# chrg127/stereomatching

Hardware: AMD Instinct MI355X
Metric: Mpixel-disparities/s (higher is better)
Workload: dtype u32 bit-packed edges, i32 counts

## Files before the change

stereomatching_amd/csrc/sm_match_bs_kernel.h:

```cpp

#pragma once
#include "sm_internal.h"

#ifndef SM_BS_TU
#error "define SM_BS_TU (a token naming the translation unit) before including this header"
#endif
#define SM_BS_CAT2(a, b) a##b
#define SM_BS_CAT(a, b) SM_BS_CAT2(a, b)

#define SM_BS_WAVES 2

#ifdef SM_STAMPS
static __device__ unsigned long long *g_sm_stamps;
int SM_BS_CAT(sm_bs_set_stamps_, SM_BS_TU)(void *buf)
{
    return hipMemcpyToSymbol(HIP_SYMBOL(g_sm_stamps), &buf, sizeof buf) == hipSuccess ? 0 : SM_ERR_HIP;
}
#define SM_STAMP(slot)                                                                          \
    do {                                                                                        \
        if ((threadIdx.x & 63) == 0 && g_sm_stamps) {                   \
            const size_t wg_ = (((size_t)blockIdx.z * gridDim.y + blockIdx.y) * gridDim.x + blockIdx.x) \
                               * (blockDim.x >> 6) + (threadIdx.x >> 6);                        \
            g_sm_stamps[wg_ * 10 + 2 * (slot)] = __builtin_amdgcn_s_memrealtime();              \
            g_sm_stamps[wg_ * 10 + 2 * (slot) + 1] = __builtin_amdgcn_s_memtime();              \
            if ((slot) == 0)                                                                    \
                g_sm_stamps[wg_ * 10 + 8] = ((unsigned long long)__builtin_amdgcn_s_getreg(63508) << 32) | \
                                            (unsigned)__builtin_amdgcn_s_getreg(63492);         \
        }                                                                                       \
    } while (0)
#else
#define SM_STAMP(slot) do { } while (0)
#endif

template <int IMM>
__device__ __forceinline__ u32 bop(u32 a, u32 b, u32 c)
{
    return __builtin_amdgcn_bitop3_b32(a, b, c, IMM);
}
#define BOP_XOR3 0x96
#define BOP_MAJ 0xE8
#define BOP_BORROW 0x8E
#define BOP_SEL 0xCA
#define BOP_XOR_AND 0x28
#define BOP_UPD 0x41

__device__ __forceinline__ u32 alignbit(u32 hi, u32 lo, u32 sh)
{
    return __builtin_amdgcn_alignbit(hi, lo, sh);
}

typedef unsigned long long u64;
struct RawRow { u64 l01; u32 l2; u64 r01, r23; };
struct RawCentre { u32 l; u64 r01; u32 r2; };
typedef __attribute__((address_space(3))) const volatile u32 lds_vu32;
typedef u64 __attribute__((aligned(4))) u64a4;
typedef __attribute__((address_space(3))) const volatile u64a4 lds_vu64;
__device__ __forceinline__ void lds_issue(RawRow &o, u32 aL, u32 aR)
{
    o.l01 = *(lds_vu64 *)(uintptr_t)aL;
    o.l2 = *(lds_vu32 *)(uintptr_t)(aL + 8);
    o.r01 = *(lds_vu64 *)(uintptr_t)aR;
    o.r23 = *(lds_vu64 *)(uintptr_t)(aR + 8);
}
__device__ __forceinline__ void lds_issue(RawCentre &o, u32 aL, u32 aR)
{
    o.l = *(lds_vu32 *)(uintptr_t)aL;
    o.r01 = *(lds_vu64 *)(uintptr_t)aR;
    o.r2 = *(lds_vu32 *)(uintptr_t)(aR + 8);
}

typedef int v4i __attribute__((ext_vector_type(4)));
__device__ __forceinline__ void store_map4(i32 *p, v4i v)
{
    asm volatile("global_store_dwordx4 %0, %1, off sc1\n\ts_nop 1" : : "v"(p), "v"(v) : "memory");
}

constexpr int bits_for(int v) { int b = 0; while ((1 << b) <= v) b++; return b; }

template <int SB, int HB>
__device__ __forceinline__ void add_planes(u32 (&s)[SB], const u32 (&h)[HB])
{
    u32 c = s[0] & h[0];
    s[0] ^= h[0];
#pragma unroll
    for (int k = 1; k < SB; k++) {
        if (k < HB) {
            const u32 cn = bop<BOP_MAJ>(s[k], h[k], c);
            s[k] = bop<BOP_XOR3>(s[k], h[k], c);
            c = cn;
        } else {
            const u32 cn = k + 1 < SB ? s[k] & c : 0u;
            s[k] ^= c;
            c = cn;
        }
    }
}

#define SM_PIN() __builtin_amdgcn_sched_barrier(0)
#define SM_SYNC() do { asm volatile("s_nop 0"); SM_PIN(); } while (0)
#define BOP_ANDN 0x0C
#define BOP_ORN 0xCF
#define BOP_XNOR 0xC3

template <int N, int HB, int IT, typename XF>
__device__ __forceinline__ void count_lockstep(XF xin, u32 (&h)[IT][HB])
{
    u32 q[IT][2 * N + 2];
    int head = 0, tail = N;
#pragma unroll
    for (int w = 0; w < HB; w++) {
        u32 nx[IT][N + 1];
        int nn = 0;
#pragma unroll
        for (int adder = 0; adder < N; adder++) {
            if (tail - head >= 3) {
                u32 a[IT], b[IT], c[IT];
#pragma unroll
                for (int it = 0; it < IT; it++) {
                    const bool in0 = w == 0 && head < N, in1 = w == 0 && head + 1 < N, in2 = w == 0 && head + 2 < N;
                    a[it] = in0 ? xin(it, in0 ? head : 0) : q[it][head];
                    b[it] = in1 ? xin(it, in1 ? head + 1 : 0) : q[it][head + 1];
                    c[it] = in2 ? xin(it, in2 ? head + 2 : 0) : q[it][head + 2];
                }
#pragma unroll
                for (int it = 0; it < IT; it++) { q[it][tail] = bop<BOP_XOR3>(a[it], b[it], c[it]); SM_PIN(); }
#pragma unroll
                for (int it = 0; it < IT; it++) { nx[it][nn] = bop<BOP_MAJ>(a[it], b[it], c[it]); SM_PIN(); }
                SM_SYNC();
                head += 3; tail++; nn++;
            }
        }
        if (tail - head == 2) {
            u32 a[IT], b[IT];
#pragma unroll
            for (int it = 0; it < IT; it++) {
                const bool in0 = w == 0 && head < N, in1 = w == 0 && head + 1 < N;
                a[it] = in0 ? xin(it, in0 ? head : 0) : q[it][head];
                b[it] = in1 ? xin(it, in1 ? head + 1 : 0) : q[it][head + 1];
            }
#pragma unroll
            for (int it = 0; it < IT; it++) { q[it][tail] = a[it] ^ b[it]; SM_PIN(); }
#pragma unroll
            for (int it = 0; it < IT; it++) { nx[it][nn] = a[it] & b[it]; SM_PIN(); }
            head += 2; tail++; nn++;
        }
#pragma unroll
        for (int it = 0; it < IT; it++) {
            const bool in0 = w == 0 && head < N;
            h[it][w] = tail - head == 1 ? (in0 ? xin(it, in0 ? head : 0) : q[it][head]) : 0u;
        }
        head = 0; tail = 0;
#pragma unroll
        for (int i = 0; i < N + 1; i++)
            if (i < nn) {
#pragma unroll
                for (int it = 0; it < IT; it++) q[it][tail] = nx[it][i];
                tail++;
            }
    }
}

template <int SB, int HB, int GS, int DS>
__device__ __forceinline__ void add_lockstep(u32 (&S)[DS][SB], int dd0, const u32 (&h)[GS][HB])
{
    u32 c[GS];
#pragma unroll
    for (int g = 0; g < GS; g++) { c[g] = S[dd0 + g][0] & h[g][0]; SM_PIN(); }
#pragma unroll
    for (int g = 0; g < GS; g++) { S[dd0 + g][0] ^= h[g][0]; SM_PIN(); }
#pragma unroll
    for (int k = 1; k < SB; k++) {
        u32 cn[GS];
#pragma unroll
        for (int g = 0; g < GS; g++) {
            if (k + 1 < SB) { cn[g] = k < HB ? bop<BOP_MAJ>(S[dd0 + g][k], h[g][k], c[g]) : (S[dd0 + g][k] & c[g]); SM_PIN(); }
            else cn[g] = 0;
        }
#pragma unroll
        for (int g = 0; g < GS; g++) {
            if (k < HB) S[dd0 + g][k] = bop<BOP_XOR3>(S[dd0 + g][k], h[g][k], c[g]);
            else S[dd0 + g][k] ^= c[g];
            SM_PIN();
        }
#pragma unroll
        for (int g = 0; g < GS; g++) c[g] = cn[g];
        SM_SYNC();
    }
}

template <int SB, int HB, int GS, int DS>
__device__ __forceinline__ void addsub_lockstep(u32 (&S)[DS][SB], int dd0, const u32 (&hn)[GS][HB],
                                                const u32 (&ho)[GS][HB])
{
    u32 dl[GS][HB], b[GS];
#pragma unroll
    for (int g = 0; g < GS; g++) { b[g] = bop<BOP_ANDN>(hn[g][0], ho[g][0], 0u); SM_PIN(); }
#pragma unroll
    for (int g = 0; g < GS; g++) { dl[g][0] = hn[g][0] ^ ho[g][0]; SM_PIN(); }
#pragma unroll
    for (int k = 1; k < HB; k++) {
#pragma unroll
        for (int g = 0; g < GS; g++) { dl[g][k] = bop<BOP_XOR3>(hn[g][k], ho[g][k], b[g]); SM_PIN(); }
#pragma unroll
        for (int g = 0; g < GS; g++) { b[g] = bop<BOP_BORROW>(hn[g][k], ho[g][k], b[g]); SM_PIN(); }
        SM_SYNC();
    }
    u32 c[GS];
#pragma unroll
    for (int g = 0; g < GS; g++) { c[g] = S[dd0 + g][0] & dl[g][0]; SM_PIN(); }
#pragma unroll
    for (int g = 0; g < GS; g++) { S[dd0 + g][0] ^= dl[g][0]; SM_PIN(); }
#pragma unroll
    for (int k = 1; k < SB; k++) {
        u32 cn[GS];
#pragma unroll
        for (int g = 0; g < GS; g++) {
            const u32 a = k < HB ? dl[g][k] : b[g];
            if (k + 1 < SB) { cn[g] = bop<BOP_MAJ>(S[dd0 + g][k], a, c[g]); SM_PIN(); } else cn[g] = 0;
        }
#pragma unroll
        for (int g = 0; g < GS; g++) {
            const u32 a = k < HB ? dl[g][k] : b[g];
            S[dd0 + g][k] = bop<BOP_XOR3>(S[dd0 + g][k], a, c[g]); SM_PIN();
        }
#pragma unroll
        for (int g = 0; g < GS; g++) c[g] = cn[g];
        SM_SYNC();
    }
}

template <int V> struct IntTag { static constexpr int value = V; };

template <int CTRL>
__device__ __forceinline__ u32 dpp(u32 v)
{
    return (u32)__builtin_amdgcn_update_dpp(0, (int)v, CTRL, 0xf, 0xf, true);
}

template <int K>
__device__ __forceinline__ u32 from_partner(u32 v)
{
    if (K == 0) return dpp<0xB1>(v);
    if (K == 1) return dpp<0x4E>(v);
    if (K == 2) return dpp<0x141>(v);
    if (K == 3) return dpp<0x140>(v);
    return (u32)__shfl_xor((int)v, 1 << K);
}


template <int N, int DS, bool FULLD, bool GHOST, bool CAP2 = false, bool DUO = false>
__global__ __launch_bounds__(DUO ? 128 : 64, SM_BS_WAVES) void k_match_bs(const u32 *__restrict__ ext,
                                                 i32 *__restrict__ web, i32 *__restrict__ best,
                                                 const MatchGeom g)
{
    constexpr int HALF = N / 2;
    constexpr int HB = bits_for(N);
    constexpr int SB = bits_for(N * N);
    constexpr int AB = DS == 16 ? 4 : DS == 8 ? 3 : 2;
    constexpr int ABMAX = AB + 6;
    static_assert(SB <= 16, "window counts are moved through two byte lanes");
    static_assert((1 << SB) - 1 > N * N, "the all-ones marker must not be a real count");
    static_assert(N + DS - 1 + 31 < 96, "right window must fit three words");

    extern __shared__ __attribute__((aligned(16))) u32 lds[];
    if (CAP2) asm volatile("" ::: "v175");
    if (web == nullptr) return;
    const int tid = DUO ? (int)(threadIdx.x & 63u) : (int)threadIdx.x;
    const int wv = DUO ? __builtin_amdgcn_readfirstlane((int)(threadIdx.x >> 6)) : 0;
    const int pair = blockIdx.z;
    SM_STAMP(0);
    const unsigned slot_parity = __builtin_amdgcn_s_getreg(63492) & 1;
    unsigned long long clk = __builtin_amdgcn_s_memtime();
    constexpr unsigned PATTERN = DS == 16 ? 0xF0F0F0F0u : 0xAAAAAAAAu;
    const unsigned long long clk0 = clk;
#define SM_SLICE_PRIO()                                                               \
    do {                                                                              \
        const unsigned unit_ = (unsigned)((clk - clk0) >> 14) & 31u;                  \
        if (((PATTERN >> unit_) ^ slot_parity) & 1) __builtin_amdgcn_s_setprio(3);    \
        else __builtin_amdgcn_s_setprio(0);                                           \
    } while (0)
#define SM_SLICE_READ() do { clk = __builtin_amdgcn_s_memtime(); } while (0)
    int tile_x, tile_y;
    sm_xcd_tile(g.tiles_x, g.tiles_y, tile_x, tile_y);
    const int tx0 = tile_x * g.tw;
    const int ty0 = tile_y * (DUO ? 2 * g.tile_h : g.tile_h);
    const int plw = g.plw, prw = g.prw, nsr = g.nsr;
    const u32 *extL = ext + (size_t)pair * 2 * g.ext_image_words;
    const u32 *extR = extL + g.ext_image_words;
    u32 *pL = lds;
    u32 *pR = pL + nsr * plw;

    {
        const int wx0 = tx0 >> 5;
        const int per_row = plw + prw;
        for (int it = threadIdx.x; it < nsr * per_row; it += DUO ? 128 : 64) {
            const int row = it / per_row, k = it - row * per_row;
            const bool is_r = k >= plw;
            const int kk = is_r ? k - plw : k;
            const u32 v = (is_r ? extR : extL)[(size_t)(ty0 + row) * g.ext_words + wx0 + kk];
            if (is_r) pR[row * prw + kk] = v; else pL[row * plw + kk] = v;
        }
    }
    __syncthreads();
    SM_STAMP(1);

    const int s = tid & (g.nl - 1);
    const int wi = tid >> g.log2nl;
    const int d0 = s * DS;
    const int x0 = tx0 + 32 * wi;
    const int bL = SM_PADT + 32 * wi - HALF, bR = bL + d0;
    const int wL = bL >> 5, shL = bL & 31, wR = bR >> 5, shR = bR & 31;
    const int bRc = SM_PADT + 32 * wi + d0;
    const int wRc = bRc >> 5, shRc = bRc & 31;
    const int wLc = 1 + wi;

    u32 cvv[N];
    if (GHOST) {
        const int lo = min(64, max(0, HALF - x0)), hi = min(64, max(0, g.w + HALF - x0));
        const unsigned long long below_hi = hi >= 64 ? ~0ull : (1ull << hi) - 1ull;
        const unsigned long long below_lo = lo >= 64 ? ~0ull : (1ull << lo) - 1ull;
        const unsigned long long cm = hi > lo ? below_hi & ~below_lo : 0ull;
        const u32 c0 = (u32)cm, c1 = (u32)(cm >> 32);
#pragma unroll
        for (int i = 0; i < N; i++) cvv[i] = i ? alignbit(c1, c0, i) : c0;
    }
    u32 dvalid = (1u << DS) - 1u;
    if (!FULLD) {
        const int dlim = g.D - d0;
        dvalid = dlim >= DS ? (1u << DS) - 1u : (dlim <= 0 ? 0u : ((1u << dlim) - 1u));
    }

    u32 S[DS][SB];
#pragma unroll
    for (int dd = 0; dd < DS; dd++)
#pragma unroll
        for (int k = 0; k < SB; k++) S[dd][k] = 0;

    struct RowViews { u32 lv[N]; u32 rw[3]; };
    auto load_views = [&](int srow, RowViews &v) {
        const u32 *rl = pL + srow * plw + wL;
        const u32 *rr = pR + srow * prw + wR;
        const u32 l0 = alignbit(rl[1], rl[0], shL), l1 = alignbit(rl[2], rl[1], shL);
#pragma unroll
        for (int k = 0; k < 3; k++) v.rw[k] = alignbit(rr[k + 1], rr[k], shR);
#pragma unroll
        for (int i = 0; i < N; i++) v.lv[i] = i ? alignbit(l1, l0, i) : l0;
    };
    auto views_of = [&](const RawRow &q, RowViews &v) {
        const u32 a0 = (u32)q.l01, a1 = (u32)(q.l01 >> 32), a2 = q.l2;
        const u32 r0 = (u32)q.r01, r1 = (u32)(q.r01 >> 32), r2 = (u32)q.r23, r3 = (u32)(q.r23 >> 32);
        const u32 l0 = alignbit(a1, a0, shL), l1 = alignbit(a2, a1, shL);
        v.rw[0] = alignbit(r1, r0, shR); v.rw[1] = alignbit(r2, r1, shR); v.rw[2] = alignbit(r3, r2, shR);
#pragma unroll
        for (int i = 0; i < N; i++) v.lv[i] = i ? alignbit(l1, l0, i) : l0;
    };
    auto rview = [&](const RowViews &v, int j) -> u32 {
        return (j & 31) ? alignbit(v.rw[(j >> 5) + 1], v.rw[j >> 5], j & 31) : v.rw[j >> 5];
    };

    constexpr int GW = DS >= 4 ? 4 : DS;
    constexpr int GS = 2;
    static_assert(DS % GW == 0 && DS % GS == 0, "shift groups");
    auto slide_in = [&](int srow) {
        RowViews v;
        load_views(srow, v);
        u32 rv[N + GW - 1];
#pragma unroll
        for (int m = 0; m < N - 1; m++) rv[m + GW] = rview(v, m);
#pragma unroll
        for (int dd0 = 0; dd0 < DS; dd0 += GW) {
#pragma unroll
            for (int m = 0; m < N - 1; m++) rv[m] = rv[m + GW];
#pragma unroll
            for (int m = 0; m < GW; m++) { rv[N - 1 + m] = rview(v, dd0 + N - 1 + m); SM_PIN(); }
            SM_SYNC();
            u32 h[GW][HB];
            count_lockstep<N, HB, GW>([&](int it, int i) -> u32 {
                const u32 x = GHOST ? bop<BOP_XOR_AND>(v.lv[i], rv[it + i], cvv[i]) : (v.lv[i] ^ rv[it + i]);
                SM_PIN();
                return x;
            }, h);
            add_lockstep<SB, HB, GW, DS>(S, dd0, h);
        }
    };
    auto slide_views = [&](const RowViews &vn, const RowViews &vo) {
        u32 rn[N + GS - 1], ro[N + GS - 1];
#pragma unroll
        for (int m = 0; m < N - 1; m++) { rn[m + GS] = rview(vn, m); ro[m + GS] = rview(vo, m); }
#pragma unroll
        for (int dd0 = 0; dd0 < DS; dd0 += GS) {
#pragma unroll
            for (int m = 0; m < N - 1; m++) { rn[m] = rn[m + GS]; ro[m] = ro[m + GS]; }
#pragma unroll
            for (int m = 0; m < GS; m++) {
                rn[N - 1 + m] = rview(vn, dd0 + N - 1 + m); SM_PIN();
                ro[N - 1 + m] = rview(vo, dd0 + N - 1 + m); SM_PIN();
            }
            SM_SYNC();
            u32 h[2 * GS][HB];
            count_lockstep<N, HB, 2 * GS>([&](int it, int i) -> u32 {
                const u32 l = (it & 1) ? vo.lv[i] : vn.lv[i];
                const u32 r = (it & 1) ? ro[(it >> 1) + i] : rn[(it >> 1) + i];
                const u32 x = GHOST ? bop<BOP_XOR_AND>(l, r, cvv[i]) : (l ^ r);
                SM_PIN();
                return x;
            }, h);
            u32 hn[GS][HB], ho[GS][HB];
#pragma unroll
            for (int gq = 0; gq < GS; gq++)
#pragma unroll
                for (int k = 0; k < HB; k++) { hn[gq][k] = h[2 * gq][k]; ho[gq][k] = h[2 * gq + 1][k]; }
            addsub_lockstep<SB, HB, GS, DS>(S, dd0, hn, ho);
            SM_SYNC();
        }
    };

    const int mid = DUO ? min(ty0 + g.tile_h, g.h) : 0;
    const int sgn = DUO ? (wv ? 1 : -1) : 1;
    const int y0 = DUO ? (wv ? mid : mid - 1) : ty0;
    const int c0 = DUO ? y0 - ty0 + HALF : HALF;
    const int rows_out = DUO ? (wv ? min(ty0 + 2 * g.tile_h, g.h) - mid : mid - ty0)
                             : min(g.tile_h, g.h - ty0);

    SM_SLICE_PRIO();
    if (DUO) {
#pragma unroll 1
        for (int e = 0; e <= HALF; e++) {
        if (e == HALF) {
        constexpr int DH = DS / 2, XP = DH * SB / 2;
        static_assert(DS % 2 == 0 && (DH * SB) % 2 == 0, "exchange halves");
        typedef u32 v2u __attribute__((ext_vector_type(2)));
        v2u *xq = reinterpret_cast<v2u *>(lds + g.xm_off - XP * 128) + tid;
        auto exchange = [&](auto own_tag) {
            constexpr int OWN = decltype(own_tag)::value, OTH = 1 - OWN;
            v2u *slot_own = xq + OWN * XP * 64, *slot_oth = xq + OTH * XP * 64;
#pragma unroll
            for (int j = 0; j < XP; j++) {
                const int p = 2 * j, q = 2 * j + 1;
                const v2u v = {S[OTH * DH + p / SB][p % SB], S[OTH * DH + q / SB][q % SB]};
                slot_oth[j * 64] = v;
            }
            __syncthreads();
#pragma unroll
            for (int dd = 0; dd < DH; dd += 2) {
                u32 o[2][SB];
#pragma unroll
                for (int j = 0; j < SB; j++) {
                    const int p = 2 * j, q = 2 * j + 1;
                    const v2u v = slot_own[(dd * SB / 2 + j) * 64];
                    o[p / SB][p % SB] = v.x;
                    o[q / SB][q % SB] = v.y;
                }
                add_planes<SB, SB>(S[OWN * DH + dd], o[0]);
                add_planes<SB, SB>(S[OWN * DH + dd + 1], o[1]);
#pragma unroll
                for (int j = 0; j < SB; j++) {
                    const int p = 2 * j, q = 2 * j + 1;
                    const v2u v = {S[OWN * DH + dd + p / SB][p % SB], S[OWN * DH + dd + q / SB][q % SB]};
                    slot_own[(dd * SB / 2 + j) * 64] = v;
                }
            }
            __syncthreads();
#pragma unroll
            for (int j = 0; j < XP; j++) {
                const int p = 2 * j, q = 2 * j + 1;
                const v2u v = slot_oth[j * 64];
                S[OTH * DH + p / SB][p % SB] = v.x;
                S[OTH * DH + q / SB][q % SB] = v.y;
            }
        };
        if (wv) exchange(IntTag<1>{}); else exchange(IntTag<0>{});
        }
        slide_in(c0 + sgn * e);
        }
        if (rows_out <= 0) return;
    } else {
#pragma unroll 1
        for (int e = 0; e < N; e++) slide_in(e);
    }
    SM_SLICE_READ();
    SM_STAMP(2);

    u32 *xm_base = lds + g.xm_off - ((DUO && wv) ? g.xm_words : 0);
    u32 *xm_wbase = xm_base + (s & 3) * ((SB + AB + 3) / 4) * 256;
    const u32 xm_wunit = (u32)(wi * (g.nl >> 2) + (s >> 2) + 2 * (s & 3));
    const u32 ldsL = (u32)(uintptr_t)pL, ldsR = (u32)(uintptr_t)pR;
    const u32 sL = (u32)(sgn * 4 * plw), sR = (u32)(sgn * 4 * prw);
    u32 aNewL = ldsL + 4u * wL + sL * (HALF + 1) + 4u * plw * c0, aNewR = ldsR + 4u * wR + sR * (HALF + 1) + 4u * prw * c0;
    u32 aCenL = ldsL + 4u * wLc + 4u * plw * c0, aCenR = ldsR + 4u * wRc + 4u * prw * c0;
    RawRow qn, qo;
    RawCentre qc;
    lds_issue(qc, aCenL, aCenR);
    if (!DUO || rows_out > 1) {
        lds_issue(qn, aNewL, aNewR);
        lds_issue(qo, aNewL - sL * N, aNewR - sR * N);
    }
#pragma unroll 1
    for (int t = 0;;) {
        SM_SLICE_PRIO();
        const int y = y0 + sgn * t;
        const u32 lc = qc.l;
        const u32 c0_ = (u32)qc.r01, c1_ = (u32)(qc.r01 >> 32), c2_ = qc.r2;
        const u32 rc0 = alignbit(c1_, c0_, shRc), rc1 = alignbit(c2_, c1_, shRc);

        u32 B[SB], arg[ABMAX];
#pragma unroll
        for (int k = 0; k < ABMAX; k++) arg[k] = 0;
        {
            constexpr int Q = 4, QS = DS / Q;
            constexpr int AQ = AB - 2;
            u32 Bq[Q][SB], aq[Q][AQ > 0 ? AQ : 1];
#pragma unroll
            for (int i = 0; i < QS; i++) {
                u32 upd[Q];
                u32 rcd[Q];
#pragma unroll
                for (int qd = 0; qd < Q; qd++) {
                    const int dd = qd * QS + i;
                    rcd[qd] = dd ? alignbit(rc1, rc0, dd) : rc0; SM_PIN();
                }
                SM_SYNC();
                if (i == 0) {
#pragma unroll
                    for (int qd = 0; qd < Q; qd++) {
                        upd[qd] = bop<BOP_XNOR>(lc, rcd[qd], 0u); SM_PIN();
                        if (!FULLD) { upd[qd] &= (u32)__builtin_amdgcn_sbfe((int)dvalid, qd * QS + i, 1); SM_PIN(); }
                    }
#pragma unroll
                    for (int k = 0; k < SB; k++)
#pragma unroll
                        for (int qd = 0; qd < Q; qd++) { Bq[qd][k] = bop<BOP_ORN>(upd[qd], S[qd * QS + i][k], 0u); SM_PIN(); }
#pragma unroll
                    for (int a = 0; a < AQ; a++)
#pragma unroll
                        for (int qd = 0; qd < Q; qd++) aq[qd][a] = 0;
                } else {
                    u32 bw[Q];
#pragma unroll
                    for (int k = 0; k < SB; k++)
#pragma unroll
                        for (int qd = 0; qd < Q; qd++) {
                            bw[qd] = bop<BOP_BORROW>(Bq[qd][k], S[qd * QS + i][k], k ? bw[qd] : 0u); SM_PIN();
                            if (qd == Q - 1 && (k & 1)) SM_SYNC();
                        }
#pragma unroll
                    for (int qd = 0; qd < Q; qd++) {
                        upd[qd] = bop<BOP_UPD>(lc, rcd[qd], bw[qd]); SM_PIN();
                        if (!FULLD) { upd[qd] &= (u32)__builtin_amdgcn_sbfe((int)dvalid, qd * QS + i, 1); SM_PIN(); }
                    }
#pragma unroll
                    for (int k = 0; k < SB; k++)
#pragma unroll
                        for (int qd = 0; qd < Q; qd++) {
                            Bq[qd][k] = bop<BOP_SEL>(upd[qd], S[qd * QS + i][k], Bq[qd][k]); SM_PIN();
                            if (qd == Q - 1 && (k & 1)) SM_SYNC();
                        }
#pragma unroll
                    for (int a = 0; a < AQ; a++)
#pragma unroll
                        for (int qd = 0; qd < Q; qd++) {
                            if ((i >> a) & 1) aq[qd][a] |= upd[qd]; else aq[qd][a] = bop<BOP_ANDN>(upd[qd], aq[qd][a], 0u);
                            SM_PIN();
                        }
                }
            }
            u32 bwm[2] = {0, 0};
#pragma unroll
            for (int k = 0; k < SB; k++)
#pragma unroll
                for (int m = 0; m < 2; m++) {
                    bwm[m] = bop<BOP_BORROW>(Bq[2 * m][k], Bq[2 * m + 1][k], k ? bwm[m] : 0u); SM_PIN();
                }
            u32 Bh[2][SB], ah[2][AQ + 1];
            u32 bwf = 0;
#pragma unroll
            for (int k = 0; k < SB; k++) {
#pragma unroll
                for (int m = 0; m < 2; m++) { Bh[m][k] = bop<BOP_SEL>(bwm[m], Bq[2 * m][k], Bq[2 * m + 1][k]); SM_PIN(); }
                if (k < AQ) {
#pragma unroll
                    for (int m = 0; m < 2; m++) { ah[m][k] = bop<BOP_SEL>(bwm[m], aq[2 * m][k], aq[2 * m + 1][k]); SM_PIN(); }
                }
                if (k > 0) { bwf = bop<BOP_BORROW>(Bh[0][k - 1], Bh[1][k - 1], k > 1 ? bwf : 0u); SM_PIN(); }
            }
#pragma unroll
            for (int k = SB; k < AQ; k++)
#pragma unroll
                for (int m = 0; m < 2; m++) { ah[m][k] = bop<BOP_SEL>(bwm[m], aq[2 * m][k], aq[2 * m + 1][k]); SM_PIN(); }
            ah[0][AQ] = ~bwm[0]; SM_PIN();
            ah[1][AQ] = ~bwm[1]; SM_PIN();
            bwf = bop<BOP_BORROW>(Bh[0][SB - 1], Bh[1][SB - 1], SB > 1 ? bwf : 0u); SM_PIN();
#pragma unroll
            for (int k = 0; k < SB; k++) { B[k] = bop<BOP_SEL>(bwf, Bh[0][k], Bh[1][k]); SM_PIN(); }
#pragma unroll
            for (int k = 0; k <= AQ; k++) { arg[k] = bop<BOP_SEL>(bwf, ah[0][k], ah[1][k]); SM_PIN(); }
            arg[AQ + 1] = ~bwf; SM_PIN();
        }

        auto emit_pixels = [&](u32 (&B)[SB], u32 (&arg)[ABMAX], int xw, int yy, int pfirst, int per, int pstep) {
            const int cw = per < 4 ? per : 4;
            const u32 cmask = (1u << cw) - 1u;
            u32 allone = B[0];
#pragma unroll
            for (int k = 1; k < SB; k++) allone &= B[k];
            u32 dm1 = (u32)(g.D - 1);
            asm volatile("" : "+s"(dm1));
#pragma unroll
            for (int k = 0; k < ABMAX; k++) {
                if (k >= AB && k >= AB + g.log2nl) continue;
                arg[k] = bop<BOP_SEL>(allone, (u32)-(i32)((dm1 >> k) & 1u), arg[k]);
            }
            for (int c = 0, p0 = pfirst; c < per; c += 4, p0 += pstep) {
                u32 bb = 0, bhi = 0, alo = 0, ahi = 0;
                if (best) {
#pragma unroll
                    for (int k = 0; k < SB; k++) {
                        const u32 sp = __umul24((B[k] >> p0) & cmask, 0x204081u) & 0x01010101u;
                        if (k < 8) bb += sp << k; else bhi += sp << (k - 8);
                    }
                }
#pragma unroll
                for (int k = 0; k < ABMAX; k++) {
                    if (k >= AB && k >= AB + g.log2nl) continue;
                    const u32 sp = __umul24((arg[k] >> p0) & cmask, 0x204081u) & 0x01010101u;
                    if (k < 8) alo += sp << k; else ahi += sp << (k - 8);
                }
                const u32 none = __umul24((allone >> p0) & cmask, 0x204081u) & 0x01010101u;
                i32 wv[4], bv[4];
#pragma unroll
                for (int q = 0; q < 4; q++) {
                    const bool no = (none >> (8 * q)) & 1u;
                    int taps = N * N;
                    if (GHOST) {
                        const int x = xw + p0 + q;
                        const int cols = min(g.w - 1, x + HALF) - max(0, x - HALF) + 1;
                        const int rws = min(g.h - 1, yy + HALF) - max(0, yy - HALF) + 1;
                        taps = cols * rws;
                    }
                    const i32 a = (i32)(((alo >> (8 * q)) & 255u) | (((ahi >> (8 * q)) & 255u) << 8));
                    wv[q] = a + 1;
                    bv[q] = no ? 0 : taps - (i32)(((bb >> (8 * q)) & 255u) | (((bhi >> (8 * q)) & 255u) << 8));
                }
                const int x = xw + p0;
                const size_t o = ((size_t)pair * g.h + yy) * g.w + x;
                const bool vec = cw == 4 && g.vec_ok && x + 4 <= g.w;
                if (g.web_bytes == 4) {
                    if (vec) {
                        const v4i wq = {wv[0], wv[1], wv[2], wv[3]};
                        store_map4(web + o, wq);
                    } else {
#pragma unroll
                        for (int q = 0; q < 4; q++)
                            if (q < cw && x + q < g.w) web[o + q] = wv[q];
                    }
                } else if (g.web_bytes == 1) {
                    u8 *web8 = reinterpret_cast<u8 *>(web);
                    if (vec) {
                        u32 pk = 0;
#pragma unroll
                        for (int q = 0; q < 4; q++) pk |= (u32)(wv[q] & 255) << (8 * q);
                        __builtin_nontemporal_store(pk, reinterpret_cast<u32 *>(web8 + o));
                    } else {
#pragma unroll
                        for (int q = 0; q < 4; q++)
                            if (q < cw && x + q < g.w) web8[o + q] = (u8)wv[q];
                    }
                } else {
                    unsigned short *web16 = reinterpret_cast<unsigned short *>(web);
                    if (vec) {
                        typedef u32 v2u __attribute__((ext_vector_type(2)));
                        const v2u pk = {(u32)wv[0] | ((u32)wv[1] << 16), (u32)wv[2] | ((u32)wv[3] << 16)};
                        __builtin_nontemporal_store(pk, reinterpret_cast<v2u *>(web16 + o));
                    } else {
#pragma unroll
                        for (int q = 0; q < 4; q++)
                            if (q < cw && x + q < g.w) web16[o + q] = (unsigned short)wv[q];
                    }
                }
                if (best) {
                    if (vec) {
                        const v4i bq = {bv[0], bv[1], bv[2], bv[3]};
                        store_map4(best + o, bq);
                    } else {
#pragma unroll
                        for (int q = 0; q < 4; q++)
                            if (q < cw && x + q < g.w) best[o + q] = bv[q];
                    }
                }
            }
        };

#define SM_MERGE(K, me, NA)                                                            \
        {                                                                              \
            u32 pb[SB], pa[NA];                                                        \
            _Pragma("unroll") for (int k = 0; k < SB; k++) pb[k] = from_partner<K>(B[k]);      \
            _Pragma("unroll") for (int k = 0; k < NA; k++) pa[k] = from_partner<K>(arg[k]);    \
            SM_PIN(); SM_SYNC();                                                       \
            const u32 mine_high = ((me) >> K) & 1 ? 0xffffffffu : 0u;                  \
            u32 bw = mine_high;           \
            bw = ~bw;                       \
            _Pragma("unroll") for (int k = 0; k < SB; k++) bw = bop<BOP_BORROW>(pb[k], B[k], bw); \
            const u32 take = bw;                                                       \
            _Pragma("unroll") for (int k = 0; k < SB; k++) B[k] = bop<BOP_SEL>(take, pb[k], B[k]); \
            _Pragma("unroll") for (int k = 0; k < NA; k++) arg[k] = bop<BOP_SEL>(take, pa[k], arg[k]); \
            arg[NA] = take ^ mine_high;                 \
        }
        if (g.xmerge) {
            constexpr int NPL = SB + AB, NPG = (NPL + 3) / 4;
            typedef u32 v4u __attribute__((ext_vector_type(4)));
            typedef __attribute__((address_space(3))) const volatile v4u lds_vv4;
            const u32 xm_lds = (u32)(uintptr_t)xm_base;
            const int r = t & 3;
            {
                u32 pl[4 * NPG];
#pragma unroll
                for (int k = 0; k < 4 * NPG; k++) pl[k] = k < SB ? B[k] : (k < NPL ? arg[k - SB] : 0u);
                const u32 unit = (xm_wunit + 16u * (u32)r) & 63u;
#pragma unroll
                for (int pg = 0; pg < NPG; pg++) {
                    const v4u v = {pl[4 * pg], pl[4 * pg + 1], pl[4 * pg + 2], pl[4 * pg + 3]};
                    *reinterpret_cast<v4u *>(xm_wbase + pg * 256 + unit * 4) = v;
                }
            }
            if (r == 3 || t + 1 >= rows_out) {
                __builtin_amdgcn_fence(__ATOMIC_RELEASE, "wavefront");
                __builtin_amdgcn_wave_barrier();
                const int lpi = g.nl >> 2, l2lpi = g.log2nl - 2;
                const int rr = tid >> 4, wr = (tid & 15) >> l2lpi, sub = tid & (lpi - 1);
                u32 Bm[SB], am[ABMAX];
#pragma unroll
                for (int k = 0; k < ABMAX; k++) am[k] = 0;
                v4u ev[4][NPG];
#pragma unroll
                for (int j = 0; j < 4; j++) {
                    const u32 unit = ((u32)tid + 2u * j) & 63u;
#pragma unroll
                    for (int pg = 0; pg < NPG; pg++)
                        ev[j][pg] = *(lds_vv4 *)(uintptr_t)(xm_lds + 4u * (u32)((j * NPG + pg) * 256) + 16u * unit);
                }
                SM_PIN();
#pragma unroll
                for (int j = 0; j < 4; j++) {
                    u32 e[4 * NPG];
#pragma unroll
                    for (int pg = 0; pg < NPG; pg++) {
                        const v4u v = ev[j][pg];
                        e[4 * pg] = v.x; e[4 * pg + 1] = v.y; e[4 * pg + 2] = v.z; e[4 * pg + 3] = v.w;
                    }
                    if (j == 0) {
#pragma unroll
                        for (int k = 0; k < SB; k++) Bm[k] = e[k];
#pragma unroll
                        for (int k = 0; k < AB; k++) am[k] = e[SB + k];
                    } else {
                        u32 bw = 0xffffffffu;
#pragma unroll
                        for (int k = 0; k < SB; k++) bw = bop<BOP_BORROW>(e[k], Bm[k], bw);
                        const u32 take = bw;
#pragma unroll
                        for (int k = 0; k < SB; k++) Bm[k] = bop<BOP_SEL>(take, e[k], Bm[k]);
#pragma unroll
                        for (int k = 0; k < AB; k++) am[k] = bop<BOP_SEL>(take, e[SB + k], am[k]);
                        if (j & 1) am[AB] |= take; else am[AB] = bop<BOP_ANDN>(take, am[AB], 0u);
                        if (j & 2) am[AB + 1] |= take; else am[AB + 1] = bop<BOP_ANDN>(take, am[AB + 1], 0u);
                    }
                }
                {
                    u32 (&B)[SB] = Bm;
                    u32 (&arg)[ABMAX] = am;
                    if (lpi > 1) SM_MERGE(0, sub, AB + 2)
                    if (lpi > 2) SM_MERGE(1, sub, AB + 3)
                    if (lpi > 4) SM_MERGE(2, sub, AB + 4)
                }
                const int tt = t - r + rr;
                const int yy = y0 + sgn * tt;
                if (rr <= r && yy < g.h && yy >= 0) {
                    const int per = 32 >> l2lpi;
                    emit_pixels(Bm, am, tx0 + 32 * wr, yy, 4 * sub, per, 4 * lpi);
                }
                __builtin_amdgcn_wave_barrier();
            }
        } else {
            if (g.nl > 1) SM_MERGE(0, s, AB)
            if (g.nl > 2) SM_MERGE(1, s, AB + 1)
            if (g.nl > 4) SM_MERGE(2, s, AB + 2)
            if (g.nl > 8) SM_MERGE(3, s, AB + 3)
            if (g.nl > 16) SM_MERGE(4, s, AB + 4)
            if (g.nl > 32) SM_MERGE(5, s, AB + 5)
            if (y < g.h) {
                const int per = 32 >> g.log2nl;
                emit_pixels(B, arg, x0, y, s * per, per, 4);
            }
        }
#undef SM_MERGE

        SM_SYNC();
        if (++t >= rows_out) break;
        {
            RowViews vn, vo;
            views_of(qn, vn);
            views_of(qo, vo);
            aNewL += sL; aNewR += sR; aCenL += sL; aCenR += sR;
            lds_issue(qc, aCenL, aCenR);
            if (t + 1 < rows_out) {
                lds_issue(qn, aNewL, aNewR);
                lds_issue(qo, aNewL - sL * N, aNewR - sR * N);
            }
            SM_SLICE_READ();
            SM_PIN(); SM_SYNC();
            slide_views(vn, vo);
        }
    }
    SM_STAMP(3);
}


template <int N, int DS, bool CAP2, bool DUO = false>
static const void *bs_ptr4(bool fulld, bool ghost)
{
    return fulld ? (ghost ? (const void *)k_match_bs<N, DS, true, true, CAP2, DUO> : (const void *)k_match_bs<N, DS, true, false, CAP2, DUO>)
                 : (ghost ? (const void *)k_match_bs<N, DS, false, true, CAP2, DUO> : (const void *)k_match_bs<N, DS, false, false, CAP2, DUO>);
}
template <int N, int DS, bool CAPPABLE>
static const void *bs_ptr(bool fulld, bool ghost, bool cap2)
{
    if (cap2) return CAPPABLE ? bs_ptr4<N, DS, CAPPABLE>(fulld, ghost) : nullptr;
    return bs_ptr4<N, DS, false>(fulld, ghost);
}
```

Before: 11.62 million.

## Stage only warm-up rows before sync and defer remaining row loads into registers

The global-to-LDS staging loop is split. Only the rows needed for the initial window warm-up are loaded before the first barrier. Up to PB words of the remaining rows are loaded into registers so their latency overlaps the warm-up computation, then written to LDS later, at the DUO exchange barrier or before a new barrier after slide-in. The division-based index walk is also replaced with an incremental row/column walk. This adds register pressure (PB extra VGPRs) and one extra barrier in the non-DUO path.

```diff
diff --git a/stereomatching_amd/csrc/sm_match_bs_kernel.h b/stereomatching_amd/csrc/sm_match_bs_kernel.h
--- a/stereomatching_amd/csrc/sm_match_bs_kernel.h
+++ b/stereomatching_amd/csrc/sm_match_bs_kernel.h
@@ -290,19 +290,63 @@
     u32 *pL = lds;
     u32 *pR = pL + nsr * plw;
 
+    constexpr int NT = DUO ? 128 : 64;
+    constexpr int NA = DUO ? N + 1 : N;
+    constexpr int PB = DS == 16 ? 7 : 0;
+    const int mid = DUO ? min(ty0 + g.tile_h, g.h) : 0;
+    const int a0 = DUO ? mid - ty0 - 1 : 0;
+    const int per_row = plw + prw;
+    const u32 *srcL = extL + (size_t)ty0 * g.ext_words + (tx0 >> 5), *srcR = extR + (size_t)ty0 * g.ext_words + (tx0 >> 5);
+    int sq = 0, sr = NT;
+    while (sr >= per_row) { sr -= per_row; sq++; }
+    auto walk_start = [&](int &row, int &k) {
+        row = 0; k = (int)threadIdx.x;
+        while (k >= per_row) { k -= per_row; row++; }
+    };
+    auto walk_step = [&](int &row, int &k) {
+        row += sq; k += sr;
+        if (k >= per_row) { k -= per_row; row++; }
+    };
+    auto stage_load = [&](int row, int k) -> u32 {
+        return k >= plw ? srcR[(size_t)row * g.ext_words + (k - plw)] : srcL[(size_t)row * g.ext_words + k];
+    };
+    auto stage_store = [&](int row, int k, u32 v) {
+        if (k >= plw) pR[row * prw + (k - plw)] = v; else pL[row * plw + k] = v;
+    };
+    const int nrem = nsr - NA;
+    auto rem_row = [&](int r) { return r < a0 ? r : r + NA; };
     {
-        const int wx0 = tx0 >> 5;
-        const int per_row = plw + prw;
-        for (int it = threadIdx.x; it < nsr * per_row; it += DUO ? 128 : 64) {
-            const int row = it / per_row, k = it - row * per_row;
-            const bool is_r = k >= plw;
-            const int kk = is_r ? k - plw : k;
-            const u32 v = (is_r ? extR : extL)[(size_t)(ty0 + row) * g.ext_words + wx0 + kk];
-            if (is_r) pR[row * prw + kk] = v; else pL[row * plw + kk] = v;
+        int row, k;
+        for (walk_start(row, k); row < NA; walk_step(row, k)) stage_store(a0 + row, k, stage_load(a0 + row, k));
+        if (nrem * per_row > NT * PB) {
+            walk_start(row, k);
+            for (int i = 0; i < PB; i++) walk_step(row, k);
+            for (; row < nrem; walk_step(row, k)) stage_store(rem_row(row), k, stage_load(rem_row(row), k));
         }
     }
     __syncthreads();
     SM_STAMP(1);
+    u32 stg[PB > 0 ? PB : 1];
+    {
+        int row, k;
+        walk_start(row, k);
+#pragma unroll
+        for (int i = 0; i < PB; i++) {
+            stg[i] = 0;
+            if (row < nrem) stg[i] = stage_load(rem_row(row), k);
+            walk_step(row, k);
+        }
+    }
+    SM_PIN();
+    auto stage_phase_b = [&]() {
+        int row, k;
+        walk_start(row, k);
+#pragma unroll
+        for (int i = 0; i < PB; i++) {
+            if (row < nrem) stage_store(rem_row(row), k, stg[i]);
+            walk_step(row, k);
+        }
+    };
 
     const int s = tid & (g.nl - 1);
     const int wi = tid >> g.log2nl;
@@ -415,7 +459,6 @@
         }
     };
 
-    const int mid = DUO ? min(ty0 + g.tile_h, g.h) : 0;
     const int sgn = DUO ? (wv ? 1 : -1) : 1;
     const int y0 = DUO ? (wv ? mid : mid - 1) : ty0;
     const int c0 = DUO ? y0 - ty0 + HALF : HALF;
@@ -440,6 +483,7 @@
                 const v2u v = {S[OTH * DH + p / SB][p % SB], S[OTH * DH + q / SB][q % SB]};
                 slot_oth[j * 64] = v;
             }
+            stage_phase_b();
             __syncthreads();
 #pragma unroll
             for (int dd = 0; dd < DH; dd += 2) {
@@ -477,6 +521,8 @@
     } else {
 #pragma unroll 1
         for (int e = 0; e < N; e++) slide_in(e);
+        stage_phase_b();
+        __syncthreads();
     }
     SM_SLICE_READ();
     SM_STAMP(2);
```

Result: no change. 11.67 million, median of 6 (+0.4%).
